# deep-privacy/SA-toolkit

Hardware: AMD Instinct MI355X
Metric: anonymized audio seconds per wall-clock second (real-time factor), 5 s @ 16 kHz utterances (higher is better)
Workload: dtype f32 (matrix products as split-f16: hi*hi on the f16 MFMA; cross terms on the block-scaled 8-bit MFMA (weights e4m3, activations e5m2) in the ResBlock convs of stages [1, 2] = 51 % of the generator's FLOP, as two more f16 products elsewhere; f32 accumulate)

## Files before the change

### sa-toolkit_amd/csrc/fbank.hip

```cpp
#include "common.h"

namespace sat {

constexpr int FB_NFFT = 512;
constexpr int FB_WIN = 400;
constexpr int FB_SHIFT = 160;
constexpr int FB_FRAMES_PER_BLOCK = 4;

__device__ __forceinline__ float wave_sum(float v) {
#pragma unroll
  for (int off = 32; off > 0; off >>= 1) v += __shfl_xor(v, off, 64);
  return v;
}

__device__ __forceinline__ float framed_sample(const float* __restrict__ w, int n, int i) {
  constexpr int pad = FB_WIN / 2 - FB_SHIFT / 2;
  int idx;
  if (i < pad)
    idx = pad - 1 - i;
  else if (i < pad + n)
    idx = i - pad;
  else
    idx = n - 1 - (i - pad - n);
  idx = idx < 0 ? 0 : (idx >= n ? n - 1 : idx);
  return w[idx];
}

__global__ void __launch_bounds__(64 * FB_FRAMES_PER_BLOCK)
fbank_frames_kernel(const float* __restrict__ wav, float* __restrict__ raw,
                    const float* __restrict__ window, const float* __restrict__ mel,
                    const int* __restrict__ mel_lo, const int* __restrict__ mel_hi, int n, int m,
                    float scale, int n_mel) {
  __shared__ float s_re[FB_FRAMES_PER_BLOCK][FB_NFFT];
  __shared__ float s_im[FB_FRAMES_PER_BLOCK][FB_NFFT];
  __shared__ float s_twr[FB_NFFT / 2], s_twi[FB_NFFT / 2];
  __shared__ float s_pw[FB_FRAMES_PER_BLOCK][FB_NFFT / 2 + 1];

  const int lane = threadIdx.x & 63;
  const int wv = threadIdx.x >> 6;
  const int b = blockIdx.y;
  const int f = blockIdx.x * FB_FRAMES_PER_BLOCK + wv;
  const bool live = f < m;
  const float* w = wav + (size_t)b * n;

  for (int k = threadIdx.x; k < FB_NFFT / 2; k += blockDim.x) {
    float s, c;
    sincospif(-(float)k / (float)(FB_NFFT / 2), &s, &c);
    s_twr[k] = c;
    s_twi[k] = s;
  }

  float* re = s_re[wv];
  float* im = s_im[wv];
  float xv[7];
  float part = 0.f;
#pragma unroll
  for (int k = 0; k < 7; ++k) {
    const int j = lane + 64 * k;
    float v = 0.f;
    if (live && j < FB_WIN) v = framed_sample(w, n, f * FB_SHIFT + j) * scale;
    xv[k] = v;
    part += v;
  }
  const float mean = wave_sum(part) / (float)FB_WIN;
#pragma unroll
  for (int k = 0; k < 7; ++k) {
    const int j = lane + 64 * k;
    if (j < FB_WIN) re[j] = xv[k] - mean;
  }
  __syncthreads();
  float yv[8];
#pragma unroll
  for (int k = 0; k < 8; ++k) {
    const int j = lane + 64 * k;
    float v = 0.f;
    if (j < FB_WIN) {
      const float cur = re[j];
      const float prev = re[j > 0 ? j - 1 : 0];
      v = (cur - 0.97f * prev) * window[j];
    }
    yv[k] = v;
  }
  __syncthreads();
#pragma unroll
  for (int k = 0; k < 8; ++k) {
    const int j = lane + 64 * k;
    const int r = (int)(__brev((unsigned)j) >> 23);
    re[r] = yv[k];
    im[r] = 0.f;
  }
  __syncthreads();
#pragma unroll 1
  for (int s = 1; s <= 9; ++s) {
    const int half = 1 << (s - 1);
    const int tstep = FB_NFFT >> s;
#pragma unroll
    for (int k = 0; k < 4; ++k) {
      const int i = lane + 64 * k;
      const int pos = i & (half - 1);
      const int a = ((i >> (s - 1)) << s) + pos;
      const int c = a + half;
      const float wr = s_twr[pos * tstep], wi = s_twi[pos * tstep];
      const float xr = re[c], xi = im[c];
      const float tr = xr * wr - xi * wi;
      const float ti = xr * wi + xi * wr;
      const float ur = re[a], ui = im[a];
      re[a] = ur + tr;
      im[a] = ui + ti;
      re[c] = ur - tr;
      im[c] = ui - ti;
    }
    __syncthreads();
  }
  for (int k = lane; k <= FB_NFFT / 2; k += 64) {
    const float a = sqrtf(re[k] * re[k] + im[k] * im[k]);
    s_pw[wv][k] = a * a;
  }
  __syncthreads();
  if (!live) return;
  for (int mb = lane; mb < n_mel; mb += 64) {
    const float* mrow = mel + (size_t)mb * (FB_NFFT / 2 + 1);
    float acc = 0.f;
    const int lo = mel_lo[mb], hi = mel_hi[mb];
    for (int k = lo; k < hi; ++k) acc = fmaf(s_pw[wv][k], mrow[k], acc);
    raw[((size_t)b * n_mel + mb) * m + f] = logf(fmaxf(acc, 1e-6f));
  }
}

__global__ void __launch_bounds__(256) row_mean_kernel(const float* __restrict__ raw, float* __restrict__ means, int m) {
  __shared__ float s_part[4];
  const size_t row = blockIdx.x;
  const float* src = raw + row * m;
  float part = 0.f;
  for (int t = threadIdx.x; t < m; t += 256) part += src[t];
  part = wave_sum(part);
  if ((threadIdx.x & 63) == 0) s_part[threadIdx.x >> 6] = part;
  __syncthreads();
  if (threadIdx.x == 0) means[row] = (s_part[0] + s_part[1] + s_part[2] + s_part[3]) / (float)m;
}

__device__ __forceinline__ int right_pad_source(int b, int p, int pad, int B, int interleave) {
  return interleave ? (int)(((long long)b * pad + p) % B) : b;
}

__global__ void __launch_bounds__(256) cmvn_pad_kernel(const float* __restrict__ raw, const float* __restrict__ means,
                                                       float* __restrict__ out, int m, int pad, int do_cmvn,
                                                       int n_ch, int B) {
  const int row = blockIdx.x;
  const int b = row / n_ch, c = row - b * n_ch;
  const float* src = raw + (size_t)row * m;
  float* dst = out + (size_t)row * (size_t)(m + 2 * pad);
  const float mean = do_cmvn ? means[row] : 0.f;
  for (int t = threadIdx.x; t < m + pad; t += 256) {
    const int s = t < pad ? 0 : t - pad;
    dst[t] = src[s] - mean;
  }
  for (int p = threadIdx.x; p < pad; p += 256) {
    const int srow = right_pad_source(b, p, pad, B, 1) * n_ch + c;
    const float mu = do_cmvn ? means[srow] : 0.f;
    dst[pad + m + p] = raw[(size_t)srow * m + (m - 1)] - mu;
  }
}

__global__ void __launch_bounds__(256) pad_replicate_kernel(const float* __restrict__ x, float* __restrict__ y,
                                                            int T, int left, int right, int C, int B,
                                                            int interleave) {
  const int To = left + T + right;
  const int t = blockIdx.x * 256 + threadIdx.x;
  if (t >= To) return;
  const long long rows = (long long)B * C;
  for (long long row = blockIdx.y; row < rows; row += gridDim.y) {
    const int b = (int)(row / C), c = (int)(row - (long long)b * C);
    float v;
    if (t < left + T) {
      const int s = t < left ? 0 : t - left;
      v = x[(size_t)row * T + s];
    } else {
      const size_t srow = (size_t)right_pad_source(b, t - left - T, right, B, interleave) * C + c;
      v = x[srow * T + (T - 1)];
    }
    y[(size_t)row * To + t] = v;
  }
}

}

using namespace sat;

extern "C" size_t sat_fbank_workspace_bytes(int B, int n) {
  if (B <= 0 || n <= 0) return 0;
  const size_t m = (size_t)(n + FB_SHIFT / 2) / FB_SHIFT;
  return align_up((size_t)B * 128 * (m + 1) * sizeof(float), 256);
}

extern "C" int sat_fbank_cmvn_pad_f32(const float* wav, float* feats, const float* window, const float* mel,
                                      const int32_t* mel_lo, const int32_t* mel_hi, void* workspace,
                                      size_t workspace_bytes, int B, int n, float scale, int n_mel, int pad,
                                      int do_cmvn, void* stream) {
  SAT_REQUIRE(wav && feats && window && mel && mel_lo && mel_hi && workspace, "fbank: null pointer");
  SAT_REQUIRE(B > 0 && n_mel > 0 && n_mel <= 128 && pad >= 0, "fbank: bad sizes");
  SAT_REQUIRE(n >= FB_WIN, "fbank: choose a window size %d that is [2, %d]", FB_WIN, n);
  const int m = (n + FB_SHIFT / 2) / FB_SHIFT;
  SAT_REQUIRE_WORKSPACE(workspace_bytes >= (size_t)B * n_mel * (m + 1) * sizeof(float), "fbank: workspace too small");
  float* raw = (float*)workspace;
  float* means = raw + (size_t)B * n_mel * m;
  dim3 grid(ceil_div(m, FB_FRAMES_PER_BLOCK), B);
  hipLaunchKernelGGL(fbank_frames_kernel, grid, dim3(64 * FB_FRAMES_PER_BLOCK), 0, (hipStream_t)stream, wav, raw,
// ... 23 lines not shown
```

### sa-toolkit_amd/csrc/yaapt.hip

```cpp
#include <cmath>
#include <type_traits>

#include "common.h"

namespace sat {

typedef sat_yaapt_plan Plan;

constexpr int FFT_N = 8192;
constexpr int FFT_LOG = 12;
constexpr int FFT_NP = 1 << FFT_LOG;
constexpr int MAXP = 4;
constexpr int NC = 6;

__device__ __forceinline__ float wsum(float v) {
#pragma unroll
  for (int off = 32; off > 0; off >>= 1) v += __shfl_xor(v, off, 64);
  return v;
}
__device__ __forceinline__ float wmax(float v) {
#pragma unroll
  for (int off = 32; off > 0; off >>= 1) v = fmaxf(v, __shfl_xor(v, off, 64));
  return v;
}
// ... 306 lines not shown
  const float pr = (ai + bi) * 0.5f, pi = (br - ar) * 0.5f;
  const float2 w = tw[(FFT_NP - 1) + k];
  const float tr = pr * w.x - pi * w.y;
  const float ti = pr * w.y + pi * w.x;
  return hypotf(er + tr, ei + ti);
}

__global__ void __launch_bounds__(256) yaapt_stage_twiddles_kernel(const float2* __restrict__ tw, float2* __restrict__ out) {
  const int i = blockIdx.x * 256 + threadIdx.x;
  if (i >= FFT_N - 1) return;
  const int h = 1 << (31 - __clz(i + 1));
  const int p = i + 1 - h;
  out[i] = tw[p * ((FFT_N / 2) / h)];
}

__global__ void __launch_bounds__(FFT_THREADS) yaapt_nlfer_kernel(const float* __restrict__ filt, const float* __restrict__ hann,
                                                         const float2* __restrict__ tw, float* __restrict__ e_raw,
                                                         const int* __restrict__ U, const Plan P) {
  extern __shared__ __attribute__((aligned(16))) float lds[];
  float* re = lds;
  float* im = lds + FFT_NP;
  __shared__ float red[8];
  const int f = blockIdx.x, b = blockIdx.y;
  if (f >= ulen(U, b, 2, P.nframes)) return;
  const float* x = filt + ((size_t)b * 2 + 0) * P.Lz + (size_t)f * P.frame_jump;
  const int first = fft_load_packed<FFT_LOG, FFT_THREADS>(re, im, P.frame_size, [&](int j) { return x[j] * hann[j]; });
  fft_from<FFT_LOG, FFT_THREADS>(re, im, tw, first);
  if (threadIdx.x >= 256) return;
  float part = 0.f;
  for (int k = P.nl_lo + threadIdx.x; k < P.nl_hi; k += 256) part += fft_packed_mag(re, im, tw, k);
  const float tot = block_sum256(part, red);
  if (threadIdx.x == 0) e_raw[(size_t)b * P.nframes + f] = tot;
}

__global__ void __launch_bounds__(256) yaapt_energy_norm_kernel(const float* __restrict__ e_raw, float* __restrict__ energy,
                                                               int* __restrict__ vuv, const int* __restrict__ U, const Plan P) {
  __shared__ float red[8];
  const int b = blockIdx.x;
  const int nf = ulen(U, b, 2, P.nframes);
  const float* e = e_raw + (size_t)b * P.nframes;
  float part = 0.f;
  for (int f = threadIdx.x; f < nf; f += 256) part += e[f];
  const float mean = block_sum256(part, red) / (float)nf;
  for (int f = threadIdx.x; f < P.nframes; f += 256) {
    const float v = f < nf ? e[f] / mean : 0.f;
    energy[(size_t)b * P.nframes + f] = v;
    vuv[(size_t)b * P.nframes + f] = (f < nf && v > P.nlfer_thresh1) ? 1 : 0;
  }
}

constexpr int SPEC_MAGP = 5 * 256;
__global__ void __launch_bounds__(FFT_THREADS) yaapt_spec_kernel(const float* __restrict__ filt, const float* __restrict__ kaiser,
                                                        const float2* __restrict__ tw, const int* __restrict__ vuv,
                                                        float* __restrict__ magbuf, const int* __restrict__ U, const Plan P) {
  extern __shared__ __attribute__((aligned(16))) float lds[];
  float* re = lds;
  float* im = lds + FFT_NP;
  __shared__ float red[8];
  const int tid = threadIdx.x;
  const int f = blockIdx.x, b = blockIdx.y;
  const int nf = P.nframes;
  if (f >= ulen(U, b, 2, nf)) return;
  if (!vuv[(size_t)b * nf + f]) return;
  const float* x = filt + ((size_t)b * 2 + 1) * P.Lz + (size_t)f * P.frame_jump;
  float part = 0.f;
#pragma unroll
  for (int k = 0; k < 5; ++k) {
    const int j = tid + 256 * k;
    if (tid < 256 && j < P.nframe_size) part += x[j] * kaiser[j];
  }
  const float mean = block_sum256(part, red) / (float)P.nframe_size;
  const int first = fft_load_packed<FFT_LOG, FFT_THREADS>(re, im, P.nframe_size, [&](int j) { return x[j] * kaiser[j] - mean; });
  const int n_mag = P.min_shc * (P.nharm + 1) + (P.max_shc - P.min_shc) * (P.nharm + 1) + P.wl;
  fft_from<FFT_LOG, FFT_THREADS>(re, im, tw, first);
  float* mo = magbuf + ((size_t)b * nf + f) * SPEC_MAGP;
  for (int i = tid; i < n_mag; i += FFT_THREADS) mo[i] = i >= P.half_wl ? fft_packed_mag(re, im, tw, i - P.half_wl) : 0.f;
}

__global__ void __launch_bounds__(256) yaapt_spec_peaks_kernel(const float* __restrict__ magbuf, const int* __restrict__ vuv,
                                                               float* __restrict__ cand, const int* __restrict__ U, const Plan P) {
  __shared__ float mag[SPEC_MAGP];
  __shared__ float red[8];
  __shared__ float s_shc[256];
  __shared__ unsigned char s_flag[256];
  const int tid = threadIdx.x;
  const int f = blockIdx.x, b = blockIdx.y;
  const int nf = P.nframes;
  if (f >= ulen(U, b, 2, nf)) return;
  float* cp = cand + (size_t)b * 8 * nf;
  float* cm = cp + 4 * (size_t)nf;
  if (!vuv[(size_t)b * nf + f]) {
    if (tid < MAXP) { cp[(size_t)tid * nf + f] = 0.f; cm[(size_t)tid * nf + f] = 1.f; }
    return;
  }
  const int n_mag = P.min_shc * (P.nharm + 1) + (P.max_shc - P.min_shc) * (P.nharm + 1) + P.wl;
  const float* mi = magbuf + ((size_t)b * nf + f) * SPEC_MAGP;
#pragma unroll
  for (int k = 0; k < 5; ++k) {
    const int i = tid + 256 * k;
    if (i < n_mag) mag[i] = mi[i];
  }
  __syncthreads();
  const int rows = P.max_shc - P.min_shc + 1;
  float shc = 0.f;
  if (tid >= P.min_shc - 1 && tid < P.min_shc - 1 + rows) {
    const int r = tid - (P.min_shc - 1);
    float s = 0.f;
    for (int w = 0; w < P.wl; ++w) {
      float pr = mag[P.min_shc + r + w];
      for (int h = 1; h <= P.nharm; ++h) pr = pr * mag[(P.min_shc + r) * (h + 1) + w];
      s += pr;
    }
    shc = s;
  }
  const int lo = P.pk_min_lag, hi = P.pk_max_lag, c = P.pk_center;
  const bool in_rng = tid >= lo && tid <= hi;
  const float mx = block_max256(in_rng ? shc : -INFINITY, red);
  if (mx > 1e-14f) shc = shc / mx;
  s_shc[tid] = shc;
  const float avg = block_sum256(in_rng ? shc : 0.f, red) / (float)(hi - lo + 1);
  bool ispk = false;
  if (tid >= lo + c + 1 && tid <= hi - c) {
    const float v = s_shc[tid];
    if (v > s_shc[tid - 1] && v > s_shc[tid + 1] && v > P.shc_thresh2 * avg) {
      ispk = true;
      for (int i = tid - c; i < tid; ++i) ispk = ispk && (s_shc[i] < v);
      for (int i = tid + 1; i <= tid + c; ++i) ispk = ispk && (s_shc[i] <= v);
    }
  }
  s_flag[tid] = ispk ? 1 : 0;
  __syncthreads();
  if (tid != 0) return;
  float pit[MAXP], mer[MAXP];
  for (int i = 0; i < MAXP; ++i) { pit[i] = 0.f; mer[i] = 1.f; }
  bool done = avg > P.inv_shc_thresh1;
  if (!done) {
    float sp[MAXP], sm[MAXP];
    int np = 0, total = 0;
    float maxm = 0.f;
    for (int n = lo + c + 1; n <= hi - c; ++n) {
      if (!s_flag[n]) continue;
      const float m = s_shc[n];
      const float pv = (float)n * P.delta;
      ++total;
      maxm = total == 1 ? m : fmaxf(maxm, m);
      int pos = np;
      while (pos > 0 && sm[pos - 1] < m) --pos;
      if (pos < MAXP) {
        const int last = np < MAXP ? np : MAXP - 1;
        for (int i = last; i > pos; --i) { sp[i] = sp[i - 1]; sm[i] = sm[i - 1]; }
        sp[pos] = pv;
        sm[pos] = m;
        if (np < MAXP) ++np;
      }
    }
    if (total == 0) maxm = 0.f;
    if (maxm / avg < P.shc_thresh1) {
      done = true;
    } else if (np > 0) {
      for (int i = 0; i < MAXP; ++i) { pit[i] = i < np ? sp[i] : 0.f; mer[i] = i < np ? sm[i] : 0.f; }
      int k = np;
      if (pit[0] > P.f0_double) { k = k + 1 < MAXP ? k + 1 : MAXP; pit[k - 1] = pit[0] / 2.0f; mer[k - 1] = P.merit_extra; }
      if (pit[0] < P.f0_half) { k = k + 1 < MAXP ? k + 1 : MAXP; pit[k - 1] = pit[0] * 2.0f; mer[k - 1] = P.merit_extra; }
      for (int i = k; i < MAXP; ++i) { pit[i] = pit[0]; mer[i] = mer[0]; }
    }
  }
  for (int i = 0; i < MAXP; ++i) { cp[(size_t)i * nf + f] = pit[i]; cm[(size_t)i * nf + f] = mer[i]; }
}

__device__ float median_small(float* v, int k) {
  for (int i = 1; i < k; ++i) {
    const float x = v[i];
    int j = i - 1;
    while (j >= 0 && v[j] > x) { v[j + 1] = v[j]; --j; }
    v[j + 1] = x;
  }
  return v[k / 2];
}
__device__ void medfilt_par(const float* in, float* out, int n, int k) {
  const int pad = k / 2;
  for (int i = threadIdx.x; i < n; i += 64) {
    float w[7];
    for (int j = 0; j < 7; ++j) {
      const int s = i + j - pad;
      w[j] = (j < k && s >= 0 && s < n) ? in[s] : 0.f;
    }
    out[i] = median_small(w, k);
  }
}
__device__ double wsum_d(double v) {
#pragma unroll
  for (int off = 32; off > 0; off >>= 1) v += __shfl_xor(v, off, 64);
  return v;
}
__device__ float mean_par(const float* v, int n) {
  double s = 0.0;
  for (int i = threadIdx.x; i < n; i += 64) s += (double)v[i];
  return (float)(wsum_d(s) / (double)n);
}
__device__ float std_unbiased_par(const float* v, int n) {
  double s = 0.0;
  for (int i = threadIdx.x; i < n; i += 64) s += (double)v[i];
  const double m = wsum_d(s) / (double)n;
  double q = 0.0;
  for (int i = threadIdx.x; i < n; i += 64) { const double d = (double)v[i] - m; q += d * d; }
  return (float)sqrt(wsum_d(q) / (double)(n - 1));
}

__device__ __forceinline__ bool path1_takes(float cand, float best) {
  return (cand != cand) || (!(best != best) && cand <= best);
}
template <int C, class TransFn>
__device__ void path1_wave(const float* local, int ls, int T, TransFn trans, unsigned char* pred,
                           unsigned char* path_out) {
  const int lane = threadIdx.x;
  const bool act = lane < C * C;
  const int i = act ? lane / C : 0;
  const int j = act ? lane % C : 0;
  float pc = lane < C ? local[lane * ls] : 0.f;
  for (int t = 1; t < T; ++t) {
    const float pcj = __shfl(pc, j, 64);
    const float v = pcj + trans(i, j, t);
    int K = 0;
    float bv = __shfl(v, i * C, 64);
// ... 107 lines not shown
        return k1 * (0.05f * d + d * d);
      };
      path1_wave<4>(vcm, nf, nv, tr, pred, path);
      for (int t = lane; t < nv; t += 64) tb[t] = vcp[path[t] * nf + t];
      __syncthreads();
      medfilt_par(tb, ta, nv, mk);
    } else {
      for (int i = lane; i < nv; i += 64) ta[i] = 150.f;
    }
    __syncthreads();
    pitch_avg = mean_par(ta, nv);
    pitch_std = tmax(std_unbiased_par(ta, nv), pitch_avg * P.spec_pitch_min_std);
    for (int i = lane; i < nv; i += 64) spec[vidx[i]] = ta[i];
  }
  __syncthreads();
  if (lane == 0) {
    if (spec[0] < pitch_avg / 2.f) spec[0] = pitch_avg;
    if (spec[nf - 1] < pitch_avg / 2.f) spec[nf - 1] = pitch_avg;
  }
  __syncthreads();
  const int nz = compact_frames(nf, [&](int f) { return spec[f] != 0.f; }, vidx);
  __syncthreads();
  for (int i = lane; i < nz; i += 64) tb[i] = spec[vidx[i]];
  __syncthreads();
  if (nz == nf) {
    for (int f = lane; f < nf; f += 64) ta[f] = tb[f];
  } else {
    const float scale = (float)nz / (float)nf;
    for (int f = lane; f < nf; f += 64) {
      float src = fmaf(scale, (float)f + 0.5f, -0.5f);
      if (src < 0.f) src = 0.f;
      int i0 = (int)floorf(src);
      if (i0 > nz - 1) i0 = nz - 1;
      float l1 = src - (float)i0;
      l1 = fminf(fmaxf(l1, 0.f), 1.f);
      const int i1 = i0 + (i0 < nz - 1 ? 1 : 0);
      const float l0 = 1.f - l1;
      ta[f] = fmaf(l0, tb[i0], l1 * tb[i1]);
    }
  }
  __syncthreads();
  if (lane == 0 && nf >= 4) { ta[0] = ta[2]; ta[1] = ta[3]; }
  __syncthreads();
  float* out = spec_out + (size_t)b * nfs;
  for (int f = lane; f < nf; f += 64) out[f] = ta[f];
  if (lane == 0) scal[b * 4 + 0] = pitch_std;
}

__global__ void __launch_bounds__(256) yaapt_frame_means_kernel(const float* __restrict__ filt, float* __restrict__ fmean,
                                                               const int* __restrict__ U, const Plan P) {
  __shared__ float s_tail[2048];
  const int lane = threadIdx.x & 63, wave = threadIdx.x >> 6;
  const int b = blockIdx.x, sig = blockIdx.y;
  const float* x = filt + ((size_t)b * 2 + sig) * P.Lz;
  float* m = fmean + ((size_t)b * 2 + sig) * P.nframes;
  const int ov = P.tda_len - P.frame_jump;
  const int T = ulen(U, b, 3, P.tda_nframes);
  for (int k = wave; k < T; k += 4) {
    float part = 0.f;
    for (int j = ov + lane; j < P.tda_len; j += 64) part += x[(size_t)k * P.frame_jump + j];
    part = wsum(part);
    if (lane == 0) s_tail[k] = part;
  }
  __syncthreads();
  if (wave != 0) return;
  auto head = [&](int k, int j) { return (k < T && j < ov) ? x[(size_t)k * P.frame_jump + j] : 0.f; };
  float h0 = head(0, lane), h1 = head(0, lane + 64);
  float prev = 0.f;
  for (int k = 0; k < T; ++k) {
    const float n0 = head(k + 1, lane), n1 = head(k + 1, lane + 64);
    float v0 = h0, v1 = h1;
    if (k > 0) {
      if (lane < ov) v0 = v0 - prev;
      if (lane + 64 < ov) v1 = v1 - prev;
    }
    const float mean = (wsum(v0 + v1) + s_tail[k]) / (float)P.tda_len;
    if (lane == 0) m[k] = mean;
    prev = mean;
    h0 = n0;
    h1 = n1;
  }
}

__global__ void __launch_bounds__(256) yaapt_nccf_kernel(const float* __restrict__ filt, const float* __restrict__ fmean,
                                                        const float* __restrict__ spec, float* __restrict__ scal,
                                                        float* __restrict__ tp, float* __restrict__ tm,
                                                        int* __restrict__ status, const int* __restrict__ U, const Plan P) {
  __shared__ float d[1024];
  __shared__ float phi[1024];
  __shared__ float red[8];
  __shared__ int s_first;
  const int tid = threadIdx.x;
  const int k = blockIdx.x, sig = blockIdx.y, b = blockIdx.z;
  const int nf = P.nframes;
  if (k >= ulen(U, b, 2, nf)) return;
  const size_t oidx = ((size_t)b * 2 + sig) * nf + k;
  const float sp = spec[(size_t)b * nf + k];
  const float pstd = scal[b * 4 + 0];
  const float fthr = 5.0f * pstd;
  const float rlo = tmax(sp - 2.0f * pstd, P.f0_min);
  const float rhi = tmin(sp + 2.0f * pstd, P.f0_max);
  const float fa = floorf(P.fs / rhi), fb = floorf(P.fs / rlo);
  float pitch = 0.f, merit = 0.f;
  const int n = P.tda_len;
  if (!(fa != fa) && !(fb != fb)) {
    const int lag_min = (int)fa - P.nccf_center;
    const int lag_max = (int)fb + P.nccf_center;
    const int N = n - lag_max;
    if (N <= 0 || lag_min < 1) {
      if (tid == 0) atomicMin((int*)scal + b * 4 + 1, k * 4 + 2);
    } else if (lag_max < lag_min) {
      if (tid == 0) atomicMin((int*)scal + b * 4 + 1, k * 4 + 3);
    } else {
      const float* x = filt + ((size_t)b * 2 + sig) * P.Lz + (size_t)k * P.frame_jump;
      const float* fm = fmean + ((size_t)b * 2 + sig) * nf;
      const float mk = fm[k];
      const float mprev = k > 0 ? fm[k - 1] : 0.f;
      const int ov = P.tda_len - P.frame_jump;
      for (int j = tid; j < n; j += 256) {
        float v = x[j];
        if (k > 0 && j < ov) v = v - mprev;
        d[j] = v - mk;
        phi[j] = 0.f;
      }
      __syncthreads();
      float part = 0.f;
      for (int j = tid; j < N; j += 256) part += d[j] * d[j];
      const float pw = block_sum256(part, red);
      const int nl = lag_max - lag_min;
      for (int l = tid; l < nl; l += 256) {
        const float* row = d + lag_min + l;
        float n0 = 0.f, n1 = 0.f, n2 = 0.f, n3 = 0.f, q0 = 0.f, q1 = 0.f, q2 = 0.f, q3 = 0.f;
        int j = 0;
        for (; j + 4 <= N; j += 4) {
          n0 = fmaf(row[j], d[j], n0); q0 = fmaf(row[j], row[j], q0);
          n1 = fmaf(row[j + 1], d[j + 1], n1); q1 = fmaf(row[j + 1], row[j + 1], q1);
          n2 = fmaf(row[j + 2], d[j + 2], n2); q2 = fmaf(row[j + 2], row[j + 2], q2);
          n3 = fmaf(row[j + 3], d[j + 3], n3); q3 = fmaf(row[j + 3], row[j + 3], q3);
        }
        for (; j < N; ++j) { n0 = fmaf(row[j], d[j], n0); q0 = fmaf(row[j], row[j], q0); }
        const float nume = (n0 + n1) + (n2 + n3);
        const float den = (q0 + q1) + (q2 + q3);
        phi[lag_min + l] = nume / sqrtf(den * pw + 0.0f);
      }
      __syncthreads();
      const int c = P.nccf_center;
      int first = 1 << 30;
      float amax = 0.f;
      for (int i = tid; i < n; i += 256) {
        const float v = phi[i];
        amax = fmaxf(amax, v);
        if (i >= lag_min + c && i <= lag_max - c && v > phi[i - 1] && v > phi[i + 1] && v > P.nccf_thresh1)
          first = min(first, i);
      }
      amax = block_max256(amax, red);
      first = wmin_i(first);
      if (tid == 0) s_first = 1 << 30;
      __syncthreads();
      if ((tid & 63) == 0) atomicMin(&s_first, first);
      __syncthreads();
      first = s_first;
      if (first < (1 << 30)) {
        bool take = amax > P.nccf_thresh2;
        if (!take) {
          const float v = phi[first];
          take = true;
          for (int i = first - c; i < first; ++i) take = take && (phi[i] < v);
          for (int i = first + 1; i <= first + c; ++i) take = take && (phi[i] <= v);
        }
        if (take) {
          pitch = (float)((double)P.fs / (double)(first + 1));
          merit = phi[first];
          if (merit > 1.0f) merit = merit / merit;
        }
      }
    }
  }
  if (tid == 0) {
    const float diff = fabsf(pitch - sp);
    const float m1 = diff < fthr ? 1.f : 0.f;
    const float match = (1.f - diff / fthr) * m1;
    tp[oidx] = pitch;
    tm[oidx] = (P.merit_boost1 * merit) * match;
  }
}

__global__ void __launch_bounds__(64) yaapt_refine_dp_kernel(const float* __restrict__ tp, const float* __restrict__ tm,
                                                            const float* __restrict__ spec, const float* __restrict__ energy,
                                                            const int* __restrict__ vuv, float* __restrict__ f0,
                                                            const float* __restrict__ scal, int* __restrict__ status,
                                                            float* __restrict__ refined, const int* __restrict__ U, const Plan P) {
  extern __shared__ __attribute__((aligned(16))) float lds[];
  const int lane = threadIdx.x;
  const int b = blockIdx.x;
  const int nfs = P.nframes;
  const int nf = ulen(U, b, 2, nfs);
  if (lane == 0) {
    const int key = ((const int*)scal)[b * 4 + 1];
    if (key != 0x7fffffff) atomicMax(&status[b], key & 3);
  }
  float* rp = lds;
  float* rm = rp + NC * (size_t)nf;
  float* ta = rm + NC * (size_t)nf;
  float* en = ta + nf;
  unsigned char* pred = (unsigned char*)(en + nf);
  unsigned char* path = pred + NC * (size_t)nf;
  const float* tp1 = tp + ((size_t)b * 2 + 0) * nfs;
  const float* tp2 = tp + ((size_t)b * 2 + 1) * nfs;
  const float* tm1 = tm + ((size_t)b * 2 + 0) * nfs;
  const float* tm2 = tm + ((size_t)b * 2 + 1) * nfs;
  const float* sp = spec + (size_t)b * nfs;
  const int* vv = vuv + (size_t)b * nfs;
  const int nt = ulen(U, b, 3, P.tda_nframes);
  for (int k = lane; k < nf; k += 64) {
    en[k] = energy[(size_t)b * nfs + k];
    float p[NC] = {0.f, 0.f, 0.f, 0.f, 0.f, 0.f}, m[NC] = {0.f, 0.f, 0.f, 0.f, 0.f, 0.f};
    if (k < nt) { p[0] = tp1[k]; m[0] = tm1[k]; p[3] = tp2[k]; m[3] = tm2[k]; }
    int ord[NC];
    for (int i = 0; i < NC; ++i) {
      int pos = i;
      while (pos > 0) {
        const float a = m[ord[pos - 1]], c = m[i];
        const bool a_nan = a != a, c_nan = c != c;
        const bool c_before_a = c_nan ? false : (a_nan ? true : (c > a));
        if (!c_before_a) break;
        ord[pos] = ord[pos - 1];
        --pos;
      }
      ord[pos] = i;
    }
    float ms[NC];
    {
      float t[NC];
      for (int i = 0; i < NC; ++i) t[i] = m[i];
      for (int i = 1; i < NC; ++i) {
        const float x = t[i];
        int j = i - 1;
        while (j >= 0 && ((t[j] != t[j]) ? !(x != x) : (x == x && t[j] > x))) { t[j + 1] = t[j]; --j; }
        t[j + 1] = x;
      }
      for (int i = 0; i < NC; ++i) ms[i] = t[NC - 1 - i];
    }
    for (int i = 0; i < NC; ++i) { rp[i * nf + k] = p[ord[i]]; rm[i * nf + k] = ms[i]; }
  }
// ... 63 lines not shown
extern "C" size_t sat_yaapt_workspace_bytes(const sat_yaapt_plan* plan, int B) {
  if (!plan || B <= 0) return 0;
  return align_up(yaapt_ws_floats(*plan, B) * sizeof(float), 256);
}

static int yaapt_run(const sat_yaapt_plan* plan, const float* wav, const int32_t* U, float* f0, int32_t* status,
                     const float* hann, const float* kaiser, const float* twiddle, void* workspace,
                     size_t workspace_bytes, int B, void* stream) {
  SAT_REQUIRE(plan && wav && f0 && status && hann && kaiser && twiddle && workspace, "yaapt: null pointer");
  const Plan& P = *plan;
  SAT_REQUIRE(B > 0 && P.n > 0, "yaapt: empty batch");
  SAT_REQUIRE(P.nfft == FFT_N, "yaapt: fft_length %d not supported (8192 only)", P.nfft);
  SAT_REQUIRE(P.maxpeaks == MAXP && P.maxcands * 2 == NC, "yaapt: shc_maxpeaks/nccf_maxcands must be 4/3");
  SAT_REQUIRE(P.nharm >= 1 && P.nharm <= 7, "yaapt: shc_numharms out of range");
  SAT_REQUIRE(P.frame_size > 15, "Frame length value %d is too short.", P.frame_size);
  SAT_REQUIRE(P.frame_size < 2048, "Frame length value %d exceeds the limit.", P.frame_size);
  SAT_REQUIRE(P.nframe_size <= 5 * 256 && P.frame_size <= FFT_N, "yaapt: frame_length too long for the spectral kernel");
  SAT_REQUIRE(P.nl_lo >= 0 && P.nl_hi <= FFT_NP, "yaapt: NLFER bins %d..%d outside the half spectrum", P.nl_lo, P.nl_hi);
  SAT_REQUIRE(P.max_shc <= 256 && P.pk_max_lag + 1 < 256 && P.pk_min_lag + P.pk_center + 1 >= 1 &&
                  P.pk_min_lag - 0 >= 0, "yaapt: SHC range out of the 256-bin kernel window");
  SAT_REQUIRE(P.min_shc * (P.nharm + 1) + (P.max_shc - P.min_shc) * (P.nharm + 1) + P.wl <= 5 * 256,
              "yaapt: SHC harmonics exceed the spectral kernel's magnitude window");
  SAT_REQUIRE(P.tda_len <= 1024 && P.tda_len > P.frame_jump && P.tda_len - P.frame_jump <= 128,
              "yaapt: tda_frame_length / frame_space combination not supported");
  SAT_REQUIRE(P.median_value >= 1 && P.median_value <= 7 && (P.median_value & 1), "yaapt: median_value must be odd <= 7");
  SAT_REQUIRE(P.nframes >= 4 && P.nframes <= 2048, "yaapt: %d frames not supported (4..2048, i.e. up to ~40 s)", P.nframes);
  SAT_REQUIRE(P.tda_nframes == P.nframes, "yaapt: tda frame count differs from the analysis frame count");
  SAT_REQUIRE(P.nframe_size + (P.nframes - 1) * P.frame_jump >= P.L,
              "yaapt: frame_space too long for frame_length: the last spectral frame ends at sample %d of the %d padded ones "
              "(the reference fails on the negative zero extension of spec_track)", P.nframe_size + (P.nframes - 1) * P.frame_jump, P.L);
  SAT_REQUIRE(P.L == P.n + 2 * P.pad && P.Lz >= P.L && P.Lz >= P.nframe_size + (P.nframes - 1) * P.frame_jump,
              "yaapt: plan lengths inconsistent (L = n + 2 pad, Lz covers the padded signal and the last spectral frame)");
  SAT_REQUIRE_WORKSPACE(workspace_bytes >= sat_yaapt_workspace_bytes(plan, B), "yaapt: workspace too small");
  hipStream_t s = (hipStream_t)stream;
  const size_t nf = P.nframes;
  float* w = (float*)workspace;
  float* filt = w;            w += (size_t)B * 2 * P.Lz;
  float* e_raw = w;           w += (size_t)B * nf;
  float* energy = w;          w += (size_t)B * nf;
  int* vuv = (int*)w;         w += (size_t)B * nf;
  float* cand = w;            w += (size_t)B * 8 * nf;
  float* spec = w;            w += (size_t)B * nf;
  float* scal = w;            w += (size_t)B * 4;
  float* fmean = w;           w += (size_t)B * 2 * nf;
  float* tp = w;              w += (size_t)B * 2 * nf;
  float* tm = w;              w += (size_t)B * 2 * nf;
  float* refined = w;         w += (size_t)B * 2 * NC * nf;
  float* magbuf = w;          w += (size_t)B * nf * SPEC_MAGP;
  w += (4 - ((uintptr_t)w / 4) % 4) % 4;
  float2* stw = (float2*)w;   w += 2 * FFT_N;
  const float2* tw = (const float2*)twiddle;
  SAT_HIP(hipMemsetAsync(status, 0, sizeof(int32_t) * B, s));

  const bool pf_vec = (P.n % 4 == 0) && (P.pad % 4 == 0) && (P.Lz % 4 == 0) && (((uintptr_t)wav & 15) == 0) && (((uintptr_t)filt & 15) == 0);
  SAT_REQUIRE((size_t)32 * P.n * 4 < ((size_t)1 << 31) && (size_t)64 * P.Lz * 4 < ((size_t)1 << 31), "yaapt: utterance too long for the prefilter's 31-bit row offsets");
  if (pf_vec) hipLaunchKernelGGL(yaapt_prefilter_kernel<true>, dim3((B + 31) / 32), dim3(PF_THREADS), 0, s, wav, filt, U, P, B);
  else hipLaunchKernelGGL(yaapt_prefilter_kernel<false>, dim3((B + 31) / 32), dim3(PF_THREADS), 0, s, wav, filt, U, P, B);
  SAT_LAUNCH_CHECK("yaapt_prefilter_kernel");
  const size_t fft_lds = 2 * FFT_NP * sizeof(float);
  static std::atomic<uint64_t> attr_done{0};
  int dev;
  if (attr_needed_on_current_device(attr_done, &dev)) {
    SAT_HIP(hipFuncSetAttribute((const void*)yaapt_nlfer_kernel, hipFuncAttributeMaxDynamicSharedMemorySize, (int)fft_lds));
    SAT_HIP(hipFuncSetAttribute((const void*)yaapt_spec_kernel, hipFuncAttributeMaxDynamicSharedMemorySize, (int)fft_lds));
    SAT_HIP(hipFuncSetAttribute((const void*)yaapt_spec_post_kernel, hipFuncAttributeMaxDynamicSharedMemorySize, 160 * 1024));
    SAT_HIP(hipFuncSetAttribute((const void*)yaapt_refine_dp_kernel, hipFuncAttributeMaxDynamicSharedMemorySize, 160 * 1024));
    attr_done_on_device(attr_done, dev);
  }
  hipLaunchKernelGGL(yaapt_stage_twiddles_kernel, dim3(FFT_N / 256), dim3(256), 0, s, tw, stw);
  SAT_LAUNCH_CHECK("yaapt_stage_twiddles_kernel");
  hipLaunchKernelGGL(yaapt_nlfer_kernel, dim3(P.nframes, B), dim3(FFT_THREADS), fft_lds, s, filt, hann, stw, e_raw, U, P);
  SAT_LAUNCH_CHECK("yaapt_nlfer_kernel");
  hipLaunchKernelGGL(yaapt_energy_norm_kernel, dim3(B), dim3(256), 0, s, e_raw, energy, vuv, U, P);
  SAT_LAUNCH_CHECK("yaapt_energy_norm_kernel");
  hipLaunchKernelGGL(yaapt_spec_kernel, dim3(P.nframes, B), dim3(FFT_THREADS), fft_lds, s, filt, kaiser, stw, vuv, magbuf, U, P);
  SAT_LAUNCH_CHECK("yaapt_spec_kernel");
  hipLaunchKernelGGL(yaapt_spec_peaks_kernel, dim3(P.nframes, B), dim3(256), 0, s, magbuf, vuv, cand, U, P);
  SAT_LAUNCH_CHECK("yaapt_spec_peaks_kernel");
  const size_t post_lds = (size_t)nf * (4 + 4 + 3) * sizeof(float) + nf * 2 * sizeof(short) + nf * 5;
  hipLaunchKernelGGL(yaapt_spec_post_kernel, dim3(B), dim3(64), post_lds, s, cand, spec, scal, status, U, P);
  SAT_LAUNCH_CHECK("yaapt_spec_post_kernel");
  hipLaunchKernelGGL(yaapt_frame_means_kernel, dim3(B, 2), dim3(256), 0, s, filt, fmean, U, P);
  SAT_LAUNCH_CHECK("yaapt_frame_means_kernel");
  hipLaunchKernelGGL(yaapt_nccf_kernel, dim3(P.nframes, 2, B), dim3(256), 0, s, filt, fmean, spec, scal, tp, tm, status, U, P);
  SAT_LAUNCH_CHECK("yaapt_nccf_kernel");
  const size_t dp_lds = (size_t)nf * (2 * NC + 2) * sizeof(float) + nf * (NC + 1);
  hipLaunchKernelGGL(yaapt_refine_dp_kernel, dim3(B), dim3(64), dp_lds, s, tp, tm, spec, energy, vuv, f0, scal, status, refined, U, P);
  SAT_LAUNCH_CHECK("yaapt_refine_dp_kernel");
  return SAT_OK;
}

extern "C" int sat_yaapt_f32(const sat_yaapt_plan* plan, const float* wav, float* f0, int32_t* status,
                             const float* hann, const float* kaiser, const float* twiddle, void* workspace,
                             size_t workspace_bytes, int B, void* stream) {
  return yaapt_run(plan, wav, nullptr, f0, status, hann, kaiser, twiddle, workspace, workspace_bytes, B, stream);
}

extern "C" int sat_yaapt_ragged_f32(const sat_yaapt_plan* plan, const float* wav, const int32_t* utt_dims, float* f0,
                                    int32_t* status, const float* hann, const float* kaiser, const float* twiddle,
                                    void* workspace, size_t workspace_bytes, int B, void* stream) {
  SAT_REQUIRE(utt_dims, "yaapt_ragged: null utt_dims");
  return yaapt_run(plan, wav, utt_dims, f0, status, hann, kaiser, twiddle, workspace, workspace_bytes, B, stream);
}
```

Measured before the change: 15720.

## Rewrite fbank FFT as wave-local radix-8 and NCCF as per-wave register-tiled kernel

The fbank kernel replaces its nine-stage LDS radix-2 FFT, which needed block barriers between stages, with three radix-8 passes done in registers. Data moves between passes through padded LDS using wave-local waitcnt syncs, and twiddles are stored per stage. The YAAPT NCCF kernel now gives each frame/signal pair a single wave that computes lag correlations in register tiles with packed float2 FMAs, replacing block-wide reductions with wave reductions. The spectral peak flags become ballot bitmasks scanned with ffs. Wave-level syncs replace __syncthreads and rely on LDS regions being private to each wave, and the new code adds complexity.

```diff
diff --git a/sa-toolkit_amd/csrc/fbank.hip b/sa-toolkit_amd/csrc/fbank.hip
--- a/sa-toolkit_amd/csrc/fbank.hip
+++ b/sa-toolkit_amd/csrc/fbank.hip
@@ -6,6 +6,34 @@
 constexpr int FB_WIN = 400;
 constexpr int FB_SHIFT = 160;
 constexpr int FB_FRAMES_PER_BLOCK = 4;
+constexpr int FB_PITCH = FB_NFFT + FB_NFFT / 8;
+
+__device__ __forceinline__ void wave_lds_sync() { asm volatile("s_waitcnt lgkmcnt(0)" ::: "memory"); }
+
+template <int E>
+__device__ __forceinline__ void fft_pass(float (&xr)[8], float (&xi)[8], const float* tw_r, const float* tw_i, int r) {
+#pragma unroll
+  for (int h = 1; h <= 4; h <<= 1) {
+    float wr[4], wi[4];
+#pragma unroll
+    for (int u = 0; u < h; ++u) {
+      wr[u] = tw_r[E * h - 1 + r + E * u];
+      wi[u] = tw_i[E * h - 1 + r + E * u];
+    }
+#pragma unroll
+    for (int t = 0; t < 8; ++t) {
+      if (t & h) continue;
+      const int c = t + h, u = t & (h - 1);
+      const float tr = xr[c] * wr[u] - xi[c] * wi[u];
+      const float ti = xr[c] * wi[u] + xi[c] * wr[u];
+      const float ur = xr[t], ui = xi[t];
+      xr[t] = ur + tr;
+      xi[t] = ui + ti;
+      xr[c] = ur - tr;
+      xi[c] = ui - ti;
+    }
+  }
+}
 
 __device__ __forceinline__ float wave_sum(float v) {
 #pragma unroll
@@ -31,10 +59,9 @@
                     const float* __restrict__ window, const float* __restrict__ mel,
                     const int* __restrict__ mel_lo, const int* __restrict__ mel_hi, int n, int m,
                     float scale, int n_mel) {
-  __shared__ float s_re[FB_FRAMES_PER_BLOCK][FB_NFFT];
-  __shared__ float s_im[FB_FRAMES_PER_BLOCK][FB_NFFT];
-  __shared__ float s_twr[FB_NFFT / 2], s_twi[FB_NFFT / 2];
-  __shared__ float s_pw[FB_FRAMES_PER_BLOCK][FB_NFFT / 2 + 1];
+  __shared__ __attribute__((aligned(16))) float s_re[FB_FRAMES_PER_BLOCK][FB_PITCH];
+  __shared__ __attribute__((aligned(16))) float s_im[FB_FRAMES_PER_BLOCK][FB_PITCH];
+  __shared__ float s_twr[FB_NFFT], s_twi[FB_NFFT];
 
   const int lane = threadIdx.x & 63;
   const int wv = threadIdx.x >> 6;
@@ -43,11 +70,13 @@
   const bool live = f < m;
   const float* w = wav + (size_t)b * n;
 
-  for (int k = threadIdx.x; k < FB_NFFT / 2; k += blockDim.x) {
+  for (int e = threadIdx.x; e < FB_NFFT - 1; e += blockDim.x) {
+    const int half = 1 << (31 - __clz(e + 1));
+    const int k = (e + 1 - half) * (FB_NFFT / 2 / half);
     float s, c;
     sincospif(-(float)k / (float)(FB_NFFT / 2), &s, &c);
-    s_twr[k] = c;
-    s_twi[k] = s;
+    s_twr[e] = c;
+    s_twi[e] = s;
   }
 
   float* re = s_re[wv];
@@ -68,7 +97,7 @@
     const int j = lane + 64 * k;
     if (j < FB_WIN) re[j] = xv[k] - mean;
   }
-  __syncthreads();
+  wave_lds_sync();
   float yv[8];
 #pragma unroll
   for (int k = 0; k < 8; ++k) {
@@ -82,47 +111,48 @@
     yv[k] = v;
   }
   __syncthreads();
+  if (!live) return;
+  float xr[8], xi[8];
 #pragma unroll
   for (int k = 0; k < 8; ++k) {
-    const int j = lane + 64 * k;
-    const int r = (int)(__brev((unsigned)j) >> 23);
-    re[r] = yv[k];
-    im[r] = 0.f;
-  }
-  __syncthreads();
-#pragma unroll 1
-  for (int s = 1; s <= 9; ++s) {
-    const int half = 1 << (s - 1);
-    const int tstep = FB_NFFT >> s;
-#pragma unroll
-    for (int k = 0; k < 4; ++k) {
-      const int i = lane + 64 * k;
-      const int pos = i & (half - 1);
-      const int a = ((i >> (s - 1)) << s) + pos;
-      const int c = a + half;
-      const float wr = s_twr[pos * tstep], wi = s_twi[pos * tstep];
-      const float xr = re[c], xi = im[c];
-      const float tr = xr * wr - xi * wi;
-      const float ti = xr * wi + xi * wr;
-      const float ur = re[a], ui = im[a];
-      re[a] = ur + tr;
-      im[a] = ui + ti;
-      re[c] = ur - tr;
-      im[c] = ui - ti;
-    }
-    __syncthreads();
-  }
-  for (int k = lane; k <= FB_NFFT / 2; k += 64) {
-    const float a = sqrtf(re[k] * re[k] + im[k] * im[k]);
-    s_pw[wv][k] = a * a;
-  }
-  __syncthreads();
-  if (!live) return;
+    xr[(int)(__brev((unsigned)k) >> 29)] = yv[k];
+    xi[k] = 0.f;
+  }
+  fft_pass<1>(xr, xi, s_twr, s_twi, 0);
+  {
+    const int g = (int)(__brev((unsigned)lane) >> 26);
+    const int at = 8 * g + 8 * (g >> 3);
+    *reinterpret_cast<float4*>(re + at) = make_float4(xr[0], xr[1], xr[2], xr[3]);
+    *reinterpret_cast<float4*>(re + at + 4) = make_float4(xr[4], xr[5], xr[6], xr[7]);
+    *reinterpret_cast<float4*>(im + at) = make_float4(xi[0], xi[1], xi[2], xi[3]);
+    *reinterpret_cast<float4*>(im + at + 4) = make_float4(xi[4], xi[5], xi[6], xi[7]);
+  }
+  wave_lds_sync();
+  {
+    const int at = 72 * (lane >> 3) + (lane & 7);
+#pragma unroll
+    for (int t = 0; t < 8; ++t) { xr[t] = re[at + 8 * t]; xi[t] = im[at + 8 * t]; }
+    fft_pass<8>(xr, xi, s_twr, s_twi, lane & 7);
+#pragma unroll
+    for (int t = 0; t < 8; ++t) { re[at + 8 * t] = xr[t]; im[at + 8 * t] = xi[t]; }
+  }
+  wave_lds_sync();
+#pragma unroll
+  for (int t = 0; t < 8; ++t) { xr[t] = re[lane + 72 * t]; xi[t] = im[lane + 72 * t]; }
+  fft_pass<64>(xr, xi, s_twr, s_twi, lane);
+  wave_lds_sync();
+  float* pw = re;
+#pragma unroll
+  for (int t = 0; t < 5; ++t) {
+    const float a = sqrtf(xr[t] * xr[t] + xi[t] * xi[t]);
+    if (t < 4 || lane == 0) pw[lane + 64 * t] = a * a;
+  }
+  wave_lds_sync();
   for (int mb = lane; mb < n_mel; mb += 64) {
     const float* mrow = mel + (size_t)mb * (FB_NFFT / 2 + 1);
     float acc = 0.f;
     const int lo = mel_lo[mb], hi = mel_hi[mb];
-    for (int k = lo; k < hi; ++k) acc = fmaf(s_pw[wv][k], mrow[k], acc);
+    for (int k = lo; k < hi; ++k) acc = fmaf(pw[k], mrow[k], acc);
     raw[((size_t)b * n_mel + mb) * m + f] = logf(fmaxf(acc, 1e-6f));
   }
 }
diff --git a/sa-toolkit_amd/csrc/yaapt.hip b/sa-toolkit_amd/csrc/yaapt.hip
--- a/sa-toolkit_amd/csrc/yaapt.hip
+++ b/sa-toolkit_amd/csrc/yaapt.hip
@@ -412,7 +412,7 @@
   __shared__ float mag[SPEC_MAGP];
   __shared__ float red[8];
   __shared__ float s_shc[256];
-  __shared__ unsigned char s_flag[256];
+  __shared__ unsigned long long s_flag[4];
   const int tid = threadIdx.x;
   const int f = blockIdx.x, b = blockIdx.y;
   const int nf = P.nframes;
@@ -458,7 +458,8 @@
       for (int i = tid + 1; i <= tid + c; ++i) ispk = ispk && (s_shc[i] <= v);
     }
   }
-  s_flag[tid] = ispk ? 1 : 0;
+  const unsigned long long wave_flags = __ballot(ispk);
+  if ((tid & 63) == 0) s_flag[tid >> 6] = wave_flags;
   __syncthreads();
   if (tid != 0) return;
   float pit[MAXP], mer[MAXP];
@@ -468,8 +469,9 @@
     float sp[MAXP], sm[MAXP];
     int np = 0, total = 0;
     float maxm = 0.f;
-    for (int n = lo + c + 1; n <= hi - c; ++n) {
-      if (!s_flag[n]) continue;
+    for (int q = 0; q < 4; ++q)
+    for (unsigned long long bits = s_flag[q]; bits; bits &= bits - 1) {
+      const int n = 64 * q + __ffsll(bits) - 1;
       const float m = s_shc[n];
       const float pv = (float)n * P.delta;
       ++total;
@@ -743,16 +745,95 @@
   }
 }
 
-__global__ void __launch_bounds__(256) yaapt_nccf_kernel(const float* __restrict__ filt, const float* __restrict__ fmean,
+constexpr int NCCF_FRAMES = 2;
+typedef float nccf_v2f __attribute__((ext_vector_type(2)));
+__device__ __forceinline__ void wave_lds_sync() { asm volatile("s_waitcnt lgkmcnt(0)" ::: "memory"); }
+__host__ __device__ constexpr int nccf_wave_floats(int n) { return 3 * ((n + 3) & ~3) + 28; }
+
+template <int L>
+__device__ __forceinline__ void nccf_products(const float* d, const float* ds, float* phi, int lane, int nl, int N, int lag_min,
+                                              float pw) {
+  constexpr int G = L / 4;
+  constexpr int PG = G + 1;
+  const int a = lane & 3;
+  const int S = N >> 2;
+  for (int base = 0; base < nl; base += 16 * L) {
+    const int t0 = base + L * (lane >> 2);
+    const bool act = t0 < nl;
+    const float* p = ds + (act ? t0 : 0) + a;
+    nccf_v2f W[PG][2], an[L / 2], aq[L / 2];
+#pragma unroll
+    for (int e = 0; e < L / 2; ++e) { an[e] = (nccf_v2f){0.f, 0.f}; aq[e] = (nccf_v2f){0.f, 0.f}; }
+#pragma unroll
+    for (int g = 0; g < G; ++g) {
+      W[g][0] = (nccf_v2f){p[4 * g], p[4 * g + 1]};
+      W[g][1] = (nccf_v2f){p[4 * g + 2], p[4 * g + 3]};
+    }
+    float dnext = d[a];
+    for (int s0 = 0; s0 < S; s0 += PG) {
+#pragma unroll
+      for (int u = 0; u < PG; ++u) {
+        if (s0 + u < S) {
+          const int s = s0 + u;
+          const float* q = p + 4 * s + L;
+          W[(G + u) % PG][0] = (nccf_v2f){q[0], q[1]};
+          W[(G + u) % PG][1] = (nccf_v2f){q[2], q[3]};
+          const float dj = dnext;
+          dnext = d[4 * s + 4 + a];
+          const nccf_v2f dd = {dj, dj};
+#pragma unroll
+          for (int g = 0; g < G; ++g)
+#pragma unroll
+            for (int h = 0; h < 2; ++h) {
+              const nccf_v2f w = W[(g + u) % PG][h];
+              an[2 * g + h] = __builtin_elementwise_fma(w, dd, an[2 * g + h]);
+              aq[2 * g + h] = __builtin_elementwise_fma(w, w, aq[2 * g + h]);
+            }
+        }
+      }
+    }
+    if (a == 0) {
+      for (int j = 4 * S; j < N; ++j) {
+        const float dj = d[j];
+#pragma unroll
+        for (int e = 0; e < L; ++e) {
+          const float r = p[j + e];
+          an[e >> 1][e & 1] = fmaf(r, dj, an[e >> 1][e & 1]);
+          aq[e >> 1][e & 1] = fmaf(r, r, aq[e >> 1][e & 1]);
+        }
+      }
+    }
+    float fin_n[G], fin_d[G];
+#pragma unroll
+    for (int e = 0; e < L; ++e) {
+      float nume = an[e >> 1][e & 1], den = aq[e >> 1][e & 1];
+      nume = nume + __shfl_xor(nume, 1, 64);
+      den = den + __shfl_xor(den, 1, 64);
+      nume = nume + __shfl_xor(nume, 2, 64);
+      den = den + __shfl_xor(den, 2, 64);
+      if ((e & 3) == 0 || (e & 3) == a) { fin_n[e >> 2] = nume; fin_d[e >> 2] = den; }
+    }
+#pragma unroll
+    for (int g = 0; g < G; ++g) {
+      const int e = 4 * g + a;
+      if (act && t0 + e < nl) phi[lag_min + t0 + e] = fin_n[g] / sqrtf(fin_d[g] * pw + 0.0f);
+    }
+  }
+}
+
+__global__ void __launch_bounds__(128 * NCCF_FRAMES) yaapt_nccf_kernel(const float* __restrict__ filt, const float* __restrict__ fmean,
                                                         const float* __restrict__ spec, float* __restrict__ scal,
                                                         float* __restrict__ tp, float* __restrict__ tm,
                                                         int* __restrict__ status, const int* __restrict__ U, const Plan P) {
-  __shared__ float d[1024];
-  __shared__ float phi[1024];
-  __shared__ float red[8];
-  __shared__ int s_first;
-  const int tid = threadIdx.x;
-  const int k = blockIdx.x, sig = blockIdx.y, b = blockIdx.z;
+  extern __shared__ __attribute__((aligned(16))) float lds[];
+  const int tid = threadIdx.x & 63;
+  const int wave = threadIdx.x >> 6;
+  const int k = blockIdx.x * NCCF_FRAMES + (wave >> 1), sig = wave & 1, b = blockIdx.y;
+  const int n = P.tda_len;
+  const int n4 = (n + 3) & ~3;
+  float* d = lds + (size_t)wave * nccf_wave_floats(n);
+  float* ds = d + n4;
+  float* phi = ds + n4 + 24;
   const int nf = P.nframes;
   if (k >= ulen(U, b, 2, nf)) return;
   const size_t oidx = ((size_t)b * 2 + sig) * nf + k;
@@ -763,7 +844,6 @@
   const float rhi = tmin(sp + 2.0f * pstd, P.f0_max);
   const float fa = floorf(P.fs / rhi), fb = floorf(P.fs / rlo);
   float pitch = 0.f, merit = 0.f;
-  const int n = P.tda_len;
   if (!(fa != fa) && !(fb != fb)) {
     const int lag_min = (int)fa - P.nccf_center;
     const int lag_max = (int)fb + P.nccf_center;
@@ -778,49 +858,39 @@
       const float mk = fm[k];
       const float mprev = k > 0 ? fm[k - 1] : 0.f;
       const int ov = P.tda_len - P.frame_jump;
-      for (int j = tid; j < n; j += 256) {
+      for (int j = tid; j < n; j += 64) {
         float v = x[j];
         if (k > 0 && j < ov) v = v - mprev;
         d[j] = v - mk;
-        phi[j] = 0.f;
-      }
-      __syncthreads();
-      float part = 0.f;
-      for (int j = tid; j < N; j += 256) part += d[j] * d[j];
-      const float pw = block_sum256(part, red);
+      }
+      for (int j = tid; j < n4 + 4; j += 64) phi[j] = 0.f;
+      wave_lds_sync();
+      for (int j = tid; j < n4 + 24; j += 64) ds[j] = j + lag_min < n ? d[j + lag_min] : 0.f;
+      float pw4[4];
+#pragma unroll
+      for (int q = 0; q < 4; ++q) {
+        float part = 0.f;
+        for (int j = 64 * q + tid; j < N; j += 256) part += d[j] * d[j];
+        pw4[q] = wsum(part);
+      }
+      const float pw = (pw4[0] + pw4[1]) + (pw4[2] + pw4[3]);
+      wave_lds_sync();
       const int nl = lag_max - lag_min;
-      for (int l = tid; l < nl; l += 256) {
-        const float* row = d + lag_min + l;
-        float n0 = 0.f, n1 = 0.f, n2 = 0.f, n3 = 0.f, q0 = 0.f, q1 = 0.f, q2 = 0.f, q3 = 0.f;
-        int j = 0;
-        for (; j + 4 <= N; j += 4) {
-          n0 = fmaf(row[j], d[j], n0); q0 = fmaf(row[j], row[j], q0);
-          n1 = fmaf(row[j + 1], d[j + 1], n1); q1 = fmaf(row[j + 1], row[j + 1], q1);
-          n2 = fmaf(row[j + 2], d[j + 2], n2); q2 = fmaf(row[j + 2], row[j + 2], q2);
-          n3 = fmaf(row[j + 3], d[j + 3], n3); q3 = fmaf(row[j + 3], row[j + 3], q3);
-        }
-        for (; j < N; ++j) { n0 = fmaf(row[j], d[j], n0); q0 = fmaf(row[j], row[j], q0); }
-        const float nume = (n0 + n1) + (n2 + n3);
-        const float den = (q0 + q1) + (q2 + q3);
-        phi[lag_min + l] = nume / sqrtf(den * pw + 0.0f);
-      }
-      __syncthreads();
+      if (nl <= 64) nccf_products<4>(d, ds, phi, tid, nl, N, lag_min, pw);
+      else if (nl <= 128) nccf_products<8>(d, ds, phi, tid, nl, N, lag_min, pw);
+      else nccf_products<12>(d, ds, phi, tid, nl, N, lag_min, pw);
+      wave_lds_sync();
       const int c = P.nccf_center;
       int first = 1 << 30;
       float amax = 0.f;
-      for (int i = tid; i < n; i += 256) {
+      for (int i = lag_min + tid; i <= lag_max; i += 64) {
         const float v = phi[i];
         amax = fmaxf(amax, v);
         if (i >= lag_min + c && i <= lag_max - c && v > phi[i - 1] && v > phi[i + 1] && v > P.nccf_thresh1)
           first = min(first, i);
       }
-      amax = block_max256(amax, red);
+      amax = wmax(amax);
       first = wmin_i(first);
-      if (tid == 0) s_first = 1 << 30;
-      __syncthreads();
-      if ((tid & 63) == 0) atomicMin(&s_first, first);
-      __syncthreads();
-      first = s_first;
       if (first < (1 << 30)) {
         bool take = amax > P.nccf_thresh2;
         if (!take) {
@@ -1050,7 +1120,9 @@
   SAT_LAUNCH_CHECK("yaapt_spec_post_kernel");
   hipLaunchKernelGGL(yaapt_frame_means_kernel, dim3(B, 2), dim3(256), 0, s, filt, fmean, U, P);
   SAT_LAUNCH_CHECK("yaapt_frame_means_kernel");
-  hipLaunchKernelGGL(yaapt_nccf_kernel, dim3(P.nframes, 2, B), dim3(256), 0, s, filt, fmean, spec, scal, tp, tm, status, U, P);
+  const size_t nccf_lds = (size_t)2 * NCCF_FRAMES * nccf_wave_floats(P.tda_len) * sizeof(float);
+  hipLaunchKernelGGL(yaapt_nccf_kernel, dim3((P.nframes + NCCF_FRAMES - 1) / NCCF_FRAMES, B), dim3(128 * NCCF_FRAMES), nccf_lds, s,
+                     filt, fmean, spec, scal, tp, tm, status, U, P);
   SAT_LAUNCH_CHECK("yaapt_nccf_kernel");
   const size_t dp_lds = (size_t)nf * (2 * NC + 2) * sizeof(float) + nf * (NC + 1);
   hipLaunchKernelGGL(yaapt_refine_dp_kernel, dim3(B), dim3(64), dp_lds, s, tp, tm, spec, energy, vuv, f0, scal, status, refined, U, P);
```

Result: no change. 15820 (median of 6 runs) (+0.6%).
